# Lumina-Group/libzkp

Measured on AMD Instinct MI355X. Metric: proofs/sec (whole node) + ms/proof p50, 4096-proof mixed batch (range / equality / membership / improvement) per MI355X, higher is better.
Workload: dtype u32/u64 integer limbs (10x25.5-bit GF(2^255-19), BN254 Fq on 9x29-bit limbs in the MSM loops and 10x26-bit elsewhere, 8x32-bit Fr and scalars mod l, 2x64-bit f128)

## Files before the change

__graft_entry__.py:

```python
import ctypes
import os
import re
import subprocess
import sys

ROOT = os.path.dirname(os.path.abspath(__file__))
CSRC = os.path.join(ROOT, "libzkp_amd", "csrc")
LIB = os.path.join(ROOT, "libzkp_amd", "lib", "libzkp_hip.so")
ORACLE_LIB = os.path.join(ROOT, "oracle", "_build", "libzkp_oracle.so")
EMUL_DIR = os.path.join(ROOT, "tests", "emul")


def _newer(target, sources):
    if not os.path.exists(target):
        return False
    t = os.path.getmtime(target)
    return all(os.path.getmtime(s) <= t for s in sources)


def _run(cmd, **kw):
    print("+", " ".join(cmd), flush=True)
    subprocess.check_call(cmd, **kw)


# ... 32 lines not shown
        _run([hipcc, "--offload-arch=gfx950", "-shared", "-pthread", "-o", LIB] + objs)


def build_oracle(force=False):
    cdir = os.path.join(ROOT, "oracle", "c")
    srcs = [os.path.join(cdir, f) for f in os.listdir(cdir)] + [os.path.join(ROOT, "oracle", "Makefile")]
    if not force and _newer(ORACLE_LIB, srcs):
        return
    _run(["make", "-C", os.path.join(ROOT, "oracle"), "clean", "all"])


def build_emul(force=False):
    out = os.path.join(EMUL_DIR, "_build")
    os.makedirs(out, exist_ok=True)
    hdrs = [os.path.join(CSRC, f) for f in os.listdir(CSRC) if f.endswith(".h")]
    for name in ("emul_math", "emul_bp", "emul_bn254", "emul_g16", "emul_stark", "emul_g16_localise"):
        so, src = os.path.join(out, "lib%s.so" % name), os.path.join(EMUL_DIR, name + ".cpp")
        if not force and _newer(so, hdrs + [src]):
            continue
        _run(["g++", "-O2", "-std=c++17", "-fPIC", "-shared", "-o", so, src])


def build_abi_caller(force=False):
    src = os.path.join(ROOT, "tests", "abi", "abi_call_all.cpp")
    out = os.path.join(ROOT, "tests", "abi", "_build")
    exe = os.path.join(out, "abi_call_all")
    os.makedirs(out, exist_ok=True)
    if force or not _newer(exe, [src, os.path.join(ROOT, "include", "libzkp_hip.h"), LIB]):
        _run(["g++", "-O1", "-std=c++17", "-pthread", "-D__HIP_PLATFORM_AMD__", "-I/opt/rocm/include", src, "-o", exe, "-L" + os.path.dirname(LIB), "-lzkp_hip",
              "-L/opt/rocm/lib", "-lamdhip64", "-Wl,-rpath,$ORIGIN/../../../libzkp_amd/lib", "-Wl,-rpath,/opt/rocm/lib"])
    return exe
# ... 78 lines not shown
```

libzkp_amd/csrc/bp_steps.h:

```cpp
#pragma once
#include "fe25519.h"
#include "sc25519.h"
#include "ge25519.h"
#include "keccak.h"

namespace zkp {

constexpr uint32_t BP_N = 64;
constexpr uint32_t BASE_B = 0, BASE_BB = 1, BASE_G = 2, BASE_H = 66, NBASE = 130;
constexpr uint32_t WBITS = 10, NWIN = 26, NENT = 512, DIGW = 13, NWIN_U64 = 7, NIELS_W = 30, SUBTAB_W = NENT * NIELS_W;
constexpr uint32_t TAPE_SLOTS = 132;
constexpr uint32_t P1_V = 0, P1_A = 2, P1_NSLOTS = 260;
constexpr uint32_t P2_NSLOTS = 4;
constexpr uint32_t PR_NSLOTS = 130;
ZKP_HD constexpr uint32_t p1_s(uint32_t n) { return 3 + 2 * n; }
ZKP_HD constexpr uint32_t tape_slots(uint32_t n) { return 2 * n + 4; }
ZKP_HD constexpr uint32_t rp_bytes(uint32_t lg) { return 32 * (9 + 2 * lg); }
constexpr uint32_t GE_W = 40;
enum { SC_Y = 0, SC_Z, SC_X, SC_W, SC_U, SC_UINV, SC_T0, SC_T1, SC_T2, SC_NUM };
enum { KIND_RANGE_MIN = 0, KIND_RANGE_MAX, KIND_THRESHOLD, KIND_CONSISTENCY, KIND_BULLETPROOF, KIND_NUM };

struct BpView {
    uint32_t M;
    uint32_t n, lg;
// ... 11 lines not shown
    uint32_t* tape;
    uint32_t* gamma;
    uint32_t* d1;
    uint32_t* d2;
    uint32_t* dr;
    uint32_t* yinvpow;
    uint32_t* ypq;
    uint32_t* r0;
    uint32_t* r1;
    uint32_t* pp;
    uint32_t* ab;
    uint32_t* gh;
    uint32_t* scal;
    uint32_t* tstate;
    uint32_t* enc;
};

ZKP_HD inline sc ld_sc(const uint32_t* p, uint32_t idx, uint32_t row, uint32_t rows) {
    sc r; const uint32_t* q = p + (size_t)idx * 8 * rows + row;
    ZKP_UNROLL for (int k = 0; k < 8; k++) r.v[k] = q[(size_t)k * rows];
    return r;
}
ZKP_HD inline void st_sc(uint32_t* p, uint32_t idx, uint32_t row, uint32_t rows, const sc& s) {
    uint32_t* q = p + (size_t)idx * 8 * rows + row;
    ZKP_UNROLL for (int k = 0; k < 8; k++) q[(size_t)k * rows] = s.v[k];
}
ZKP_HD inline void st_digits_raw(uint32_t* d, uint32_t slot, uint32_t row, uint32_t rows, const sc& raw, uint32_t wbits = 0) {
    uint32_t* q = d + (size_t)slot * DIGW * rows + row;
    if (wbits == 16) {
        uint32_t pk[8]; sc_recode_signed65536(pk, raw);
// ... 123 lines not shown

ZKP_HD inline void strobe_save(const BpView& V, uint32_t job, const Strobe& s) {
    for (int i = 0; i < 50; i++) V.tstate[(size_t)i * V.M + job] = s.base[i * s.stride];
    V.tstate[(size_t)50 * V.M + job] = s.pos; V.tstate[(size_t)51 * V.M + job] = s.pos_begin;
}
ZKP_HD inline void strobe_load(const BpView& V, uint32_t job, Strobe& s) {
    for (int i = 0; i < 50; i++) s.base[i * s.stride] = V.tstate[(size_t)i * V.M + job];
    s.pos = V.tstate[(size_t)50 * V.M + job]; s.pos_begin = V.tstate[(size_t)51 * V.M + job];
}
ZKP_HD inline sc merlin_challenge_scalar(Strobe& s, const char* label, uint32_t label_len) {
    uint32_t w[16]; merlin_challenge_words(s, label, label_len, w, 16);
    return sc_from_wide(w);
}
ZKP_HD inline void merlin_append_scalar(Strobe& s, const char* label, uint32_t label_len, const sc& raw) { merlin_append_words(s, label, label_len, raw.v, 8); }

ZKP_HD inline void step_transcript1(const BpView& V, uint32_t job, Strobe& s) {
    const uint32_t M = V.M;
    switch (V.kind[job]) {
        case KIND_RANGE_MIN: merlin_init(s, "libzkp_range_min", 16); break;
        case KIND_RANGE_MAX: merlin_init(s, "libzkp_range_max", 16); break;
        case KIND_THRESHOLD: merlin_init(s, "libzkp_threshold", 16); break;
        case KIND_CONSISTENCY: merlin_init(s, "libzkp_consistency", 18); break;
        default: merlin_init(s, "libzkp_bulletproof", 18); break;
    }
    merlin_append_bytes(s, "dom-sep", 7, "rangeproof v1", 13);
    merlin_append_u64(s, "n", 1, V.n);
    merlin_append_u64(s, "m", 1, 1);
    const sc Ve = ld_sc(V.enc, 0, job, M), Ae = ld_sc(V.enc, 1, job, M), Se = ld_sc(V.enc, 2, job, M);
    merlin_append_words(s, "V", 1, Ve.v, 8);
    merlin_append_words(s, "A", 1, Ae.v, 8);
    merlin_append_words(s, "S", 1, Se.v, 8);
    const sc y = merlin_challenge_scalar(s, "y", 1);
    const sc z = merlin_challenge_scalar(s, "z", 1);
    strobe_save(V, job, s);
    st_sc(V.scal, SC_Y, job, M, y);
    st_sc(V.scal, SC_Z, job, M, z);
    const sc yinv = sc_invert(y);
    for (uint32_t h = 0; h < 2; h++) {
        const sc base = h ? yinv : y;
        sc p = sc_one();
        for (uint32_t b = 0; b < 8; b++) { st_sc(V.ypq, 16 * h + b, job, M, p); p = sc_mul(p, base); }
        sc q = sc_one();
        for (uint32_t a = 0; a < 8; a++) { st_sc(V.ypq, 16 * h + 8 + a, job, M, q); q = sc_mul(q, p); }
    }
    uint8_t* pr = V.out + V.proof_off[job];
    put_bytes(pr, Ae.v, 8); put_bytes(pr + 32, Se.v, 8);
    put_bytes(V.out + V.commit_off[job], Ve.v, 8);
}

ZKP_HD inline void step_poly(const BpView& V, uint32_t i, uint32_t job) {
    const uint32_t M = V.M;
    const sc yi = sc_mul(ld_sc(V.ypq, 8 + (i >> 3), job, M), ld_sc(V.ypq, i & 7u, job, M));
    st_sc(V.yinvpow, i, job, M, sc_mul(ld_sc(V.ypq, 24 + (i >> 3), job, M), ld_sc(V.ypq, 16 + (i & 7u), job, M)));
    const sc z = ld_sc(V.scal, SC_Z, job, M);
    const sc zz = sc_mul(z, z);
    const uint32_t bit = (uint32_t)(V.v[job] >> i) & 1u;
    const sc one = sc_one();
    const sc l0 = bit ? sc_sub(one, z) : sc_neg(z);
    const sc arz = bit ? z : sc_sub(z, one);
    const sc two_i = sc_from_u64(1ull << i);
    const sc r0 = sc_add(sc_mul(yi, arz), sc_mul(zz, two_i));
    const sc l1 = ld_sc(V.tape, 2 + i, job, M);
// ... 15 lines not shown
    }
    return t;
}
ZKP_HD inline void step_poly_sum_finish(const BpView& V, uint32_t job, const ScTriple& t) {
    const uint32_t M = V.M;
    const sc t0 = t.a, t2 = t.c, t1 = sc_sub(sc_sub(t.b, t0), t2);
    st_sc(V.scal, SC_T0, job, M, t0); st_sc(V.scal, SC_T1, job, M, t1); st_sc(V.scal, SC_T2, job, M, t2);
    st_digits(V.d2, 0, job, M, t1, V.wbits);
    st_digits(V.d2, 2, job, M, t2, V.wbits);
}
ZKP_HD inline void step_poly_sum(const BpView& V, uint32_t job) {
    ScTriple t = step_poly_sum_part(V, 0, job);
    for (uint32_t p = 1; p < 8; p++) t = triple_add(t, step_poly_sum_part(V, p, job));
    step_poly_sum_finish(V, job, t);
}
ZKP_HD inline void step_transcript2(const BpView& V, uint32_t job, Strobe& s) {
    const uint32_t M = V.M;
    strobe_load(V, job, s);
    const sc T1e = ld_sc(V.enc, 0, job, M), T2e = ld_sc(V.enc, 1, job, M);
    merlin_append_words(s, "T_1", 3, T1e.v, 8);
    merlin_append_words(s, "T_2", 3, T2e.v, 8);
    const sc x = merlin_challenge_scalar(s, "x", 1);
    const sc xx = sc_mul(x, x);
    const sc z = ld_sc(V.scal, SC_Z, job, M), zz = sc_mul(z, z);
    const sc t0 = ld_sc(V.scal, SC_T0, job, M), t1 = ld_sc(V.scal, SC_T1, job, M), t2 = ld_sc(V.scal, SC_T2, job, M);
    const sc t_x = sc_add(sc_add(t0, sc_mul(t1, x)), sc_mul(t2, xx));
    const sc t1_bl = ld_sc(V.tape, 2 + 2 * V.n, job, M), t2_bl = ld_sc(V.tape, 3 + 2 * V.n, job, M);
    const sc t_x_bl = sc_add(sc_add(sc_mul(zz, ld_sc(V.gamma, 0, job, M)), sc_mul(t1_bl, x)), sc_mul(t2_bl, xx));
    const sc e_bl = sc_add(ld_sc(V.tape, 0, job, M), sc_mul(ld_sc(V.tape, 1, job, M), x));
    const sc r_tx = sc_to_raw(t_x), r_txb = sc_to_raw(t_x_bl), r_eb = sc_to_raw(e_bl);
    merlin_append_scalar(s, "t_x", 3, r_tx);
    merlin_append_scalar(s, "t_x_blinding", 12, r_txb);
    merlin_append_scalar(s, "e_blinding", 10, r_eb);
    const sc w = merlin_challenge_scalar(s, "w", 1);
    merlin_append_bytes(s, "dom-sep", 7, "ipp v1", 6);
    merlin_append_u64(s, "n", 1, V.n);
    strobe_save(V, job, s);
    st_sc(V.scal, SC_X, job, M, x); st_sc(V.scal, SC_W, job, M, w);
    uint8_t* pr = V.out + V.proof_off[job];
    put_bytes(pr + 64, T1e.v, 8); put_bytes(pr + 96, T2e.v, 8);
    put_bytes(pr + 128, r_tx.v, 8); put_bytes(pr + 160, r_txb.v, 8); put_bytes(pr + 192, r_eb.v, 8);
}
ZKP_HD inline void step_lr_init(const BpView& V, uint32_t i, uint32_t job) {
    const uint32_t M = V.M;
    const sc z = ld_sc(V.scal, SC_Z, job, M), x = ld_sc(V.scal, SC_X, job, M);
    const uint32_t bit = (uint32_t)(V.v[job] >> i) & 1u;
    const sc l0 = bit ? sc_sub(sc_one(), z) : sc_neg(z);
    const sc a = sc_add(l0, sc_mul(ld_sc(V.tape, 2 + i, job, M), x));
    const sc b = sc_add(ld_sc(V.r0, i, job, M), sc_mul(ld_sc(V.r1, i, job, M), x));
    st_sc(V.ab, i, job, M, a); st_sc(V.ab, 64 + i, job, M, b);
}

ZKP_HD inline void step_round_prep(const BpView& V, uint32_t r, uint32_t i, uint32_t job) {
    const uint32_t M = V.M, p = V.lg - 1 - r, k = 1u << p, half = V.n >> 1;
    const uint32_t* abp = V.ab + (size_t)(r & 1) * (2 * 64 * 8) * M;
    uint32_t* abn = V.ab + (size_t)((r + 1) & 1) * (2 * 64 * 8) * M;
    sc u = sc_one(), uinv = sc_one();
// ... 22 lines not shown
    st_digits(V.dr, bit ? V.n + 2 + half + rank : 1 + half + rank, job, M, sc_mul(bx, h), V.wbits);
    if (i < k) {
        const sc ai = cur_a(i), bi = cur_b(i);
        st_sc(V.pp, i, job, M, sc_mul(ai, bx));
        st_sc(V.pp, 32 + i, job, M, sc_mul(ax, bi));
    }
}
ZKP_HD inline void step_round_sum(const BpView& V, uint32_t r, uint32_t job) {
    const uint32_t M = V.M, k = (V.n >> 1) >> r;
    sc cL = sc_zero(), cR = sc_zero();
    for (uint32_t j = 0; j < k; j++) { cL = sc_add(cL, ld_sc(V.pp, j, job, M)); cR = sc_add(cR, ld_sc(V.pp, 32 + j, job, M)); }
    const sc w = ld_sc(V.scal, SC_W, job, M);
    st_digits(V.dr, 0, job, M, sc_mul(cL, w), V.wbits);
    st_digits(V.dr, V.n + 1, job, M, sc_mul(cR, w), V.wbits);
}
ZKP_HD inline void step_transcript_round(const BpView& V, uint32_t r, uint32_t job, Strobe& s) {
    const uint32_t M = V.M;
    strobe_load(V, job, s);
    const sc Le = ld_sc(V.enc, 0, job, M), Re = ld_sc(V.enc, 1, job, M);
    merlin_append_words(s, "L", 1, Le.v, 8);
    merlin_append_words(s, "R", 1, Re.v, 8);
    const sc u = merlin_challenge_scalar(s, "u", 1);
    const sc uinv = sc_invert(u);
    uint8_t* pr = V.out + V.proof_off[job];
    put_bytes(pr + 224 + 64 * r, Le.v, 8); put_bytes(pr + 256 + 64 * r, Re.v, 8);
    if (r + 1 < V.lg) {
        strobe_save(V, job, s);
        st_sc(V.scal, SC_U, job, M, u); st_sc(V.scal, SC_UINV, job, M, uinv);
    } else {
        const uint32_t* abp = V.ab + (size_t)(V.lg & 1u) * (2 * 64 * 8) * M;
        const sc a = sc_add(sc_mul(ld_sc(abp, 0, job, M), u), sc_mul(ld_sc(abp, 1, job, M), uinv));
        const sc b = sc_add(sc_mul(ld_sc(abp, 64, job, M), uinv), sc_mul(ld_sc(abp, 65, job, M), u));
        const sc ra = sc_to_raw(a), rb = sc_to_raw(b);
        put_bytes(pr + 224 + 64 * V.lg, ra.v, 8); put_bytes(pr + 256 + 64 * V.lg, rb.v, 8);
    }
}

struct CtView {
    uint32_t C;
    const uint64_t* v; const uint32_t* seed_ix; const uint32_t* bl_ix; const uint32_t* seeds;
    uint32_t* digits;
    uint32_t wbits = 0;
};
ZKP_HD inline void step_ctask(const CtView& T, uint32_t c) {
    uint32_t seed[8]; const uint32_t* p = T.seeds + (size_t)T.seed_ix[c] * 8;
    ZKP_UNROLL for (int k = 0; k < 8; k++) seed[k] = p[k];
    const uint64_t v = T.v[c];
    st_digits_raw(T.digits, 0, c, T.C, sc_words((uint32_t)v, (uint32_t)(v >> 32), 0, 0, 0, 0, 0, 0), T.wbits);
    st_digits(T.digits, 1, c, T.C, tape_blinding(seed, T.bl_ix[c]), T.wbits);
}
// ... 40 lines not shown
```

libzkp_amd/csrc/zkp_hip.hip:

```cpp
#include <hip/hip_runtime.h>
#include <mutex>
#include <memory>
#include <algorithm>
#include <map>
#include <array>
#include <type_traits>
#include <atomic>
#include <thread>
#include <condition_variable>
#include <functional>
#include <deque>
#include <new>
#include <exception>
#include <cstring>
#include <string>
#include <vector>
#include <cstdio>
#include <cstdlib>
#include <cmath>
#include <chrono>
#include <sys/random.h>
#include "bp_layout.h"
#include "g16_steps.h"
#include "sha256_host.h"
// ... 59 lines not shown
__global__ void __launch_bounds__(TB) k_lr_init(BpView V) {
    ZKP_RAISE_PRIO();
    const uint32_t job = blockIdx.x * TB + threadIdx.x;
    if (job < V.M) step_lr_init(V, blockIdx.y, job);
}
__global__ void __launch_bounds__(TB, LAT_WAVES) k_round_prep(BpView V, uint32_t r) {
    ZKP_RAISE_PRIO();
    const uint32_t job = blockIdx.x * TB + threadIdx.x;
    if (job < V.M) step_round_prep(V, r, blockIdx.y, job);
}
__global__ void __launch_bounds__(TW, LAT_WAVES) k_round_sum(BpView V, uint32_t r) {
    ZKP_RAISE_PRIO();
    const uint32_t job = blockIdx.x * TW + threadIdx.x;
    if (job < V.M) step_round_sum(V, r, job);
}
__global__ void __launch_bounds__(TW, 1) k_transcript1(BpView V) {
    ZKP_RAISE_PRIO();
    __shared__ uint32_t lds[50 * TW];
    const uint32_t job = blockIdx.x * TW + threadIdx.x;
    Strobe s; s.base = lds + threadIdx.x; s.stride = TW; s.pos = 0; s.pos_begin = 0;
    if (job < V.M) step_transcript1(V, job, s);
}
__global__ void __launch_bounds__(TW, 1) k_transcript2(BpView V) {
    ZKP_RAISE_PRIO();
    __shared__ uint32_t lds[50 * TW];
    const uint32_t job = blockIdx.x * TW + threadIdx.x;
    Strobe s; s.base = lds + threadIdx.x; s.stride = TW; s.pos = 0; s.pos_begin = 0;
    if (job < V.M) step_transcript2(V, job, s);
}
__global__ void __launch_bounds__(TW, 1) k_transcript_round(BpView V, uint32_t r) {
    ZKP_RAISE_PRIO();
    __shared__ uint32_t lds[50 * TW];
    const uint32_t job = blockIdx.x * TW + threadIdx.x;
    Strobe s; s.base = lds + threadIdx.x; s.stride = TW; s.pos = 0; s.pos_begin = 0;
    if (job < V.M) step_transcript_round(V, r, job, s);
}
__global__ void __launch_bounds__(TW, 1) k_encode(ReduceView R, const uint32_t* sums) {
    ZKP_RAISE_PRIO();
    const uint32_t row = blockIdx.x * TW + threadIdx.x, target = blockIdx.y;
    if (row >= R.rows) return;
    sc e; ge_ristretto_encode(e.v, ld_ge(sums, target, row, R.rows));
    st_sc(R.enc, target, row, R.rows, e);
    if (R.out_off != nullptr && target == 0) put_bytes(R.out + R.out_off[row], e.v, 8);
}

struct EdMsm {
    static constexpr uint32_t ACC_W = GE_W;
    using Acc = ge;
    static __device__ __forceinline__ Acc identity() { return ge_identity(); }
    static __device__ __forceinline__ void store(uint32_t* p, uint32_t idx, uint32_t row, uint32_t rows, const Acc& a) { st_ge(p, idx, row, rows, a); }
// ... 118 lines not shown
};
constexpr uint32_t NSLOTS = 2;

struct G16State; struct StarkState; struct VfyState; struct BatchState;
struct Device {
    int index = 0, hip_dev = 0;
    std::mutex mu;
    bool ready = false;
    uint64_t generation = 0;
    int num_cu = 256;
    int msm_prio_now = 0;
    hipStream_t stream = nullptr;
    uint32_t* d_edg_table = nullptr;
    EdgGeom edg = {0, 0, 0, 0, 0};
    bool bp_ready = false;
    int edg_blocks_per_cu = 3;
    struct Family { LayoutSet p1, rd[6]; bool ready = false; };
    Family fam[4];
    LayoutSet p2, ct;
    uint32_t max_chunks = 0;
    SubBatch sub[NSLOTS];
    uint32_t next_slot = 0;
    DevPool pool;
    G16State* g16 = nullptr; StarkState* stark = nullptr; VfyState* vfy = nullptr; BatchState* batch = nullptr;
    bool profiling = false;
    struct KProf {
        std::vector<std::pair<hipEvent_t, hipEvent_t>> ev_pool; size_t ev_used = 0;
        double ms = 0; uint64_t launches = 0, adds = 0;
    };
    KProf prof[3];
// ... 290 lines not shown
    drop();
    D.edg = g;
    R.v.push_back({D.hip_dev, D.d_edg_table, 1, g});
    return 0;
}
int ensure_bp() {
    Device& D = dev();
    if (D.bp_ready) return 0;
    int rc;
    if ((rc = build_edg_table())) return rc;
    D.max_chunks = 0;
    if ((rc = upload_set(D.p2, targets_phase2((uint8_t)D.edg.nwin)))) return rc;
    if ((rc = upload_set(D.ct, targets_ctask((uint8_t)D.edg.nwin, (uint8_t)D.edg.nwin_u64)))) return rc;
    D.max_chunks = D.p2.max_chunks;
    if ((rc = ensure_family(6))) return rc;
    D.bp_ready = true;
    return 0;
}

int init_device() {
    Device& D = dev();
    if (D.ready) return 0;
    bool lazy = false;
    int rc = ed_tables_lazy(&lazy);
    if (rc) return rc;
    hipDeviceProp_t prop; HIP_TRY(hipGetDeviceProperties(&prop, D.hip_dev));
    D.num_cu = prop.multiProcessorCount > 0 ? prop.multiProcessorCount : 256;
    if (!D.stream) HIP_TRY(hipStreamCreateWithFlags(&D.stream, hipStreamNonBlocking));
    if (!lazy && (rc = ensure_bp())) return rc;
    D.ready = true;
// ... 102 lines not shown
    uint64_t* ct_off;
    int* flag;
};
size_t align_up(size_t x) { return (x + 255) & ~(size_t)255; }

size_t carve(uint8_t* base, uint32_t M, uint32_t C, uint32_t max_chunks, Ws* w) {
    size_t off = 0;
    auto take = [&](size_t bytes) { uint8_t* p = base ? base + off : nullptr; off += align_up(bytes); return p; };
    const size_t W = (size_t)8 * 4 * M;
    const size_t WD = (size_t)DIGW * 4 * M;
    Ws t{};
    t.J.v = (uint64_t*)take(8ull * M); t.J.seed_ix = (uint32_t*)take(4ull * M); t.J.proof_ix = (uint32_t*)take(4ull * M);
    t.J.bl_plus = (int32_t*)take(4ull * M); t.J.bl_minus = (int32_t*)take(4ull * M); t.J.kind = (uint8_t*)take(M);
    t.J.proof_off = (uint64_t*)take(8ull * M); t.J.commit_off = (uint64_t*)take(8ull * M);
    t.J.ct_v = (uint64_t*)take(8ull * C); t.J.ct_seed_ix = (uint32_t*)take(4ull * C); t.J.ct_bl_ix = (uint32_t*)take(4ull * C); t.J.ct_off = (uint64_t*)take(8ull * C);
    t.V.wbits = dev().edg.wbits; t.T.wbits = dev().edg.wbits;
    t.V.M = M; t.V.v = t.J.v; t.V.seed_ix = t.J.seed_ix; t.V.proof_ix = t.J.proof_ix; t.V.bl_plus = t.J.bl_plus; t.V.bl_minus = t.J.bl_minus;
    t.V.kind = t.J.kind; t.V.proof_off = t.J.proof_off; t.V.commit_off = t.J.commit_off;
    t.V.tape = (uint32_t*)take(W * TAPE_SLOTS); t.V.gamma = (uint32_t*)take(W);
    t.V.d1 = (uint32_t*)take(WD * P1_NSLOTS); t.V.d2 = (uint32_t*)take(WD * P2_NSLOTS); t.V.dr = (uint32_t*)take(WD * PR_NSLOTS);
    t.V.yinvpow = (uint32_t*)take(W * 64); t.V.ypq = (uint32_t*)take(W * 32); t.V.r0 = (uint32_t*)take(W * 64); t.V.r1 = (uint32_t*)take(W * 64);
    t.V.pp = (uint32_t*)take(W * 192); t.V.ab = (uint32_t*)take(W * 256); t.V.gh = (uint32_t*)take(W * 128);
    t.V.scal = (uint32_t*)take(W * SC_NUM); t.V.tstate = (uint32_t*)take(4ull * 52 * M); t.V.enc = (uint32_t*)take(W * 3);
    t.partial = (uint32_t*)take((size_t)max_chunks * GE_W * 4 * M);
    t.sums = (uint32_t*)take((size_t)3 * GE_W * 4 * M);
    t.T.C = C; t.T.v = t.J.ct_v; t.T.seed_ix = t.J.ct_seed_ix; t.T.bl_ix = t.J.ct_bl_ix;
    t.T.digits = (uint32_t*)take((size_t)2 * DIGW * 4 * C);
    t.ct_partial = (uint32_t*)take((size_t)(dev().ct.max_chunks ? dev().ct.max_chunks : 2) * GE_W * 4 * C);
    t.ct_enc = (uint32_t*)take((size_t)8 * 4 * C);
    t.ct_sums = (uint32_t*)take((size_t)GE_W * 4 * C);
    t.ct_off = t.J.ct_off;
// ... 35 lines not shown
    ReduceView R; R.rows = rows; R.ntargets = D.ntargets; R.partial = partial; R.target_chunk_begin = D.target_chunk_begin;
    R.enc = enc; R.out_off = out_off; R.out = out; R.corr = nullptr;
    ZKP_TRACED("k_sum_t<EdMsm>", st, launch_sum_ed(R, sums, st));
    ZKP_TRACED("k_encode", st, k_encode<<<dim3((rows + TW - 1) / TW, D.ntargets), TW, 0, st>>>(R, sums));
    return 0;
}
int msm_and_encode(const LayoutSet& S, uint32_t rows, const uint32_t* digits, uint32_t* partial, uint32_t* sums, uint32_t* enc, const uint64_t* out_off, uint8_t* out, hipStream_t st) {
    const DevLayout& D = pick_layout(S, rows);
    int rc = launch_msm(D, rows, digits, partial, st);
    if (rc) return rc;
    return launch_reduce(D, rows, partial, sums, enc, out_off, out, st);
}

int run_pipeline(const Ws& w, uint32_t M, uint32_t C, hipStream_t st, SubBatch& lane) {
    int rc;
    const dim3 gj((M + TB - 1) / TB), gw((M + TW - 1) / TW);
    const uint32_t n = w.V.n, lg = w.V.lg;
    const Device::Family& F = dev().fam[lg - 3];
    const bool forked = C != 0 && M != 0;
    if (C) {
        hipStream_t cs = forked ? lane.side : st;
        if (forked) { HIP_TRY(hipEventRecord(lane.side_go, st)); HIP_TRY(hipStreamWaitEvent(cs, lane.side_go, 0)); }
        ZKP_TRACED("k_ctask", cs, k_ctask<<<(C + TB - 1) / TB, TB, 0, cs>>>(w.T));
        if ((rc = msm_and_encode(dev().ct, C, w.T.digits, w.ct_partial, w.ct_sums, w.ct_enc, w.ct_off, w.V.out, cs))) return rc;
        if (forked) HIP_TRY(hipEventRecord(lane.side_done, cs));
    }
    if (M == 0) { HIP_TRY(hipGetLastError()); return 0; }
    ZKP_TRACED("k_tape", st, k_tape<<<dim3(gj.x, tape_slots(n) + 1), TB, 0, st>>>(w.V));
    if ((rc = msm_and_encode(F.p1, M, w.V.d1, w.partial, w.sums, w.V.enc, nullptr, nullptr, st))) return rc;
    ZKP_TRACED("k_transcript1", st, k_transcript1<<<gw, TW, 0, st>>>(w.V));
    ZKP_TRACED("k_poly", st, k_poly<<<dim3(gj.x, n), TB, 0, st>>>(w.V));
    ZKP_TRACED("k_poly_sum", st, k_poly_sum<<<(M + 7) / 8, TW, 0, st>>>(w.V));
    if ((rc = msm_and_encode(dev().p2, M, w.V.d2, w.partial, w.sums, w.V.enc, nullptr, nullptr, st))) return rc;
    ZKP_TRACED("k_transcript2", st, k_transcript2<<<gw, TW, 0, st>>>(w.V));
    ZKP_TRACED("k_lr_init", st, k_lr_init<<<dim3(gj.x, n), TB, 0, st>>>(w.V));
    for (uint32_t r = 0; r < lg; r++) {
        ZKP_TRACED("k_round_prep", st, k_round_prep<<<dim3(gj.x, n), TB, 0, st>>>(w.V, r));
        ZKP_TRACED("k_round_sum", st, k_round_sum<<<gw, TW, 0, st>>>(w.V, r));
        if ((rc = msm_and_encode(F.rd[r], M, w.V.dr, w.partial, w.sums, w.V.enc, nullptr, nullptr, st))) return rc;
        ZKP_TRACED("k_transcript_round", st, k_transcript_round<<<gw, TW, 0, st>>>(w.V, r));
    }
    if (forked) HIP_TRY(hipStreamWaitEvent(st, lane.side_done, 0));
    HIP_TRY(hipGetLastError());
    return 0;
}

__global__ void k_any_failed(const int32_t* status, uint32_t n, int* flag) {
    const uint32_t i = blockIdx.x * blockDim.x + threadIdx.x;
    if (i < n && status[i] != 0) atomicOr(flag, 1);
}

int prove_range_device_locked(uint64_t n, const uint64_t* d_value, const uint64_t* d_min, const uint64_t* d_max, uint32_t lg,
                              const uint8_t* d_seeds, uint8_t* d_out, uint64_t stride, uint32_t* d_out_len, int32_t* d_status,
                              hipStream_t st, int* any_failed, int slot_hint = -1) {
    if (n == 0) { if (any_failed) *any_failed = 0; return 0; }
// ... 234 lines not shown
    t_sel = 0;
    for (Device* d : shards) {
        std::lock_guard<std::mutex> lk(d->mu);
        if (!d->ready) continue;
        Device* prev = t_dev; t_dev = d;
        (void)hipSetDevice(d->hip_dev);
        (void)hipDeviceSynchronize();
        batch_release_all();
        g16_release_all();
        bpv_release_all();
        stark_release_all();
        d->pool.release_all();
        for (auto& sb : d->sub) release_sub(sb);
        d->msm_prio_now = 0;
        release_edg_table();
        free_set(d->p2); free_set(d->ct);
        for (auto& F : d->fam) { free_set(F.p1); for (auto& s : F.rd) free_set(s); F.ready = false; }
        trace_release();
        for (auto& K : d->prof) { for (auto& e : K.ev_pool) { (void)hipEventDestroy(e.first); (void)hipEventDestroy(e.second); } K = Device::KProf(); }
        d->g16_verify = Device::G16VerifyStats();
        (void)hipStreamDestroy(d->stream); d->stream = nullptr;
        d->ready = false; d->bp_ready = false; d->profiling = false; d->max_chunks = 0; d->next_slot = 0; d->generation++;
        t_dev = prev;
    }
} ZKP_API_CATCH_VOID

void zkp_hip_profile_enable(int on) try {
    std::vector<Device*> shards;
    { Registry& R = registry(); std::lock_guard<std::mutex> lk(R.mu); shards = R.shards; }
    for (Device* d : shards) { std::lock_guard<std::mutex> dl(d->mu); d->profiling = on != 0; }
// ... 131 lines not shown
```

Before: 329,500.

## Run Bulletproof Merlin transcripts cooperatively across 32 lanes per job

Replaces the one-thread-per-job Strobe/Keccak transcript kernels with a cooperative version. Each job's 25-lane Keccak state is spread across 32 lanes of a wave using ds_bpermute shuffles, and the scalar tails (inversions, powers, proof writes) are then done by one thread per job from shared memory. It also precomputes the fixed transcript prefix per kind and size on the host and loads it instead of re-absorbing it. This targets the serial, LDS-heavy per-thread Keccak latency in the transcript steps. In exchange it uses many more threads per job and adds block syncs and some idle lanes during the tails.

```diff
diff --git a/__graft_entry__.py b/__graft_entry__.py
--- a/__graft_entry__.py
+++ b/__graft_entry__.py
@@ -70,7 +70,7 @@
     out = os.path.join(EMUL_DIR, "_build")
     os.makedirs(out, exist_ok=True)
     hdrs = [os.path.join(CSRC, f) for f in os.listdir(CSRC) if f.endswith(".h")]
-    for name in ("emul_math", "emul_bp", "emul_bn254", "emul_g16", "emul_stark", "emul_g16_localise"):
+    for name in ("emul_math", "emul_bp", "emul_bn254", "emul_g16", "emul_stark", "emul_g16_localise", "emul_transcript_lanes"):
         so, src = os.path.join(out, "lib%s.so" % name), os.path.join(EMUL_DIR, name + ".cpp")
         if not force and _newer(so, hdrs + [src]):
             continue
diff --git a/libzkp_amd/csrc/bp_steps.h b/libzkp_amd/csrc/bp_steps.h
--- a/libzkp_amd/csrc/bp_steps.h
+++ b/libzkp_amd/csrc/bp_steps.h
@@ -3,6 +3,7 @@
 #include "sc25519.h"
 #include "ge25519.h"
 #include "keccak.h"
+#include "keccak_lanes.h"
 
 namespace zkp {
 
@@ -49,6 +50,7 @@
     uint32_t* scal;
     uint32_t* tstate;
     uint32_t* enc;
+    const uint32_t* tprefix = nullptr;
 };
 
 ZKP_HD inline sc ld_sc(const uint32_t* p, uint32_t idx, uint32_t row, uint32_t rows) {
@@ -202,9 +204,8 @@
 }
 ZKP_HD inline void merlin_append_scalar(Strobe& s, const char* label, uint32_t label_len, const sc& raw) { merlin_append_words(s, label, label_len, raw.v, 8); }
 
-ZKP_HD inline void step_transcript1(const BpView& V, uint32_t job, Strobe& s) {
-    const uint32_t M = V.M;
-    switch (V.kind[job]) {
+ZKP_HD inline void transcript_prefix(Strobe& s, uint32_t kind, uint32_t n) {
+    switch (kind) {
         case KIND_RANGE_MIN: merlin_init(s, "libzkp_range_min", 16); break;
         case KIND_RANGE_MAX: merlin_init(s, "libzkp_range_max", 16); break;
         case KIND_THRESHOLD: merlin_init(s, "libzkp_threshold", 16); break;
@@ -212,15 +213,22 @@
         default: merlin_init(s, "libzkp_bulletproof", 18); break;
     }
     merlin_append_bytes(s, "dom-sep", 7, "rangeproof v1", 13);
-    merlin_append_u64(s, "n", 1, V.n);
+    merlin_append_u64(s, "n", 1, n);
     merlin_append_u64(s, "m", 1, 1);
-    const sc Ve = ld_sc(V.enc, 0, job, M), Ae = ld_sc(V.enc, 1, job, M), Se = ld_sc(V.enc, 2, job, M);
-    merlin_append_words(s, "V", 1, Ve.v, 8);
-    merlin_append_words(s, "A", 1, Ae.v, 8);
-    merlin_append_words(s, "S", 1, Se.v, 8);
-    const sc y = merlin_challenge_scalar(s, "y", 1);
-    const sc z = merlin_challenge_scalar(s, "z", 1);
-    strobe_save(V, job, s);
+}
+constexpr uint32_t TPREFIX_W = 52, TPREFIX_N = KIND_NUM * 4;
+ZKP_HD inline uint32_t tprefix_entry(uint32_t kind, uint32_t lg) { return (kind < KIND_NUM ? kind : (uint32_t)KIND_BULLETPROOF) * 4 + (lg - 3); }
+inline void host_build_tprefix(uint32_t out[TPREFIX_N * TPREFIX_W]) {
+    for (uint32_t kind = 0; kind < KIND_NUM; kind++) for (uint32_t lg = 3; lg <= 6; lg++) {
+        uint32_t* e = out + (size_t)tprefix_entry(kind, lg) * TPREFIX_W;
+        Strobe s; s.base = e; s.stride = 1; s.pos = 0; s.pos_begin = 0;
+        transcript_prefix(s, kind, 1u << lg);
+        e[50] = s.pos; e[51] = s.pos_begin;
+    }
+}
+ZKP_HD inline void transcript1_tail(const BpView& V, uint32_t job, const uint32_t* ch) {
+    const uint32_t M = V.M;
+    const sc y = sc_from_wide(ch), z = sc_from_wide(ch + 16);
     st_sc(V.scal, SC_Y, job, M, y);
     st_sc(V.scal, SC_Z, job, M, z);
     const sc yinv = sc_invert(y);
@@ -231,9 +239,33 @@
         sc q = sc_one();
         for (uint32_t a = 0; a < 8; a++) { st_sc(V.ypq, 16 * h + 8 + a, job, M, q); q = sc_mul(q, p); }
     }
+    const sc Ve = ld_sc(V.enc, 0, job, M), Ae = ld_sc(V.enc, 1, job, M), Se = ld_sc(V.enc, 2, job, M);
     uint8_t* pr = V.out + V.proof_off[job];
     put_bytes(pr, Ae.v, 8); put_bytes(pr + 32, Se.v, 8);
     put_bytes(V.out + V.commit_off[job], Ve.v, 8);
+}
+ZKP_HD inline void step_transcript1(const BpView& V, uint32_t job, Strobe& s) {
+    const uint32_t M = V.M;
+    transcript_prefix(s, V.kind[job], V.n);
+    const sc Ve = ld_sc(V.enc, 0, job, M), Ae = ld_sc(V.enc, 1, job, M), Se = ld_sc(V.enc, 2, job, M);
+    merlin_append_words(s, "V", 1, Ve.v, 8);
+    merlin_append_words(s, "A", 1, Ae.v, 8);
+    merlin_append_words(s, "S", 1, Se.v, 8);
+    uint32_t ch[32];
+    merlin_challenge_words(s, "y", 1, ch, 16);
+    merlin_challenge_words(s, "z", 1, ch + 16, 16);
+    strobe_save(V, job, s);
+    transcript1_tail(V, job, ch);
+}
+template <class P> ZKP_HD inline void coop_transcript1_sponge(const BpView& V, uint32_t job, uint32_t* ch) {
+    const size_t M = V.M;
+    KlStrobe<P> s; kl_load(s, V.tprefix + (size_t)tprefix_entry(V.kind[job], V.lg) * TPREFIX_W, 1);
+    kl_append(s, "V", 1, KlWords{V.enc + job, M}, 32);
+    kl_append(s, "A", 1, KlWords{V.enc + 8 * M + job, M}, 32);
+    kl_append(s, "S", 1, KlWords{V.enc + 16 * M + job, M}, 32);
+    kl_challenge(s, "y", 1, (uint8_t*)ch, 64);
+    kl_challenge(s, "z", 1, (uint8_t*)(ch + 16), 64);
+    kl_save(s, V.tstate + job, M);
 }
 
 ZKP_HD inline void step_poly(const BpView& V, uint32_t i, uint32_t job) {
@@ -279,13 +311,10 @@
     for (uint32_t p = 1; p < 8; p++) t = triple_add(t, step_poly_sum_part(V, p, job));
     step_poly_sum_finish(V, job, t);
 }
-ZKP_HD inline void step_transcript2(const BpView& V, uint32_t job, Strobe& s) {
-    const uint32_t M = V.M;
-    strobe_load(V, job, s);
+ZKP_HD inline void transcript2_tail(const BpView& V, uint32_t job, const uint32_t* ch, uint32_t* raw) {
+    const uint32_t M = V.M;
     const sc T1e = ld_sc(V.enc, 0, job, M), T2e = ld_sc(V.enc, 1, job, M);
-    merlin_append_words(s, "T_1", 3, T1e.v, 8);
-    merlin_append_words(s, "T_2", 3, T2e.v, 8);
-    const sc x = merlin_challenge_scalar(s, "x", 1);
+    const sc x = sc_from_wide(ch);
     const sc xx = sc_mul(x, x);
     const sc z = ld_sc(V.scal, SC_Z, job, M), zz = sc_mul(z, z);
     const sc t0 = ld_sc(V.scal, SC_T0, job, M), t1 = ld_sc(V.scal, SC_T1, job, M), t2 = ld_sc(V.scal, SC_T2, job, M);
@@ -294,18 +323,47 @@
     const sc t_x_bl = sc_add(sc_add(sc_mul(zz, ld_sc(V.gamma, 0, job, M)), sc_mul(t1_bl, x)), sc_mul(t2_bl, xx));
     const sc e_bl = sc_add(ld_sc(V.tape, 0, job, M), sc_mul(ld_sc(V.tape, 1, job, M), x));
     const sc r_tx = sc_to_raw(t_x), r_txb = sc_to_raw(t_x_bl), r_eb = sc_to_raw(e_bl);
-    merlin_append_scalar(s, "t_x", 3, r_tx);
-    merlin_append_scalar(s, "t_x_blinding", 12, r_txb);
-    merlin_append_scalar(s, "e_blinding", 10, r_eb);
+    ZKP_UNROLL for (int k = 0; k < 8; k++) { raw[k] = r_tx.v[k]; raw[8 + k] = r_txb.v[k]; raw[16 + k] = r_eb.v[k]; }
+    st_sc(V.scal, SC_X, job, M, x);
+    uint8_t* pr = V.out + V.proof_off[job];
+    put_bytes(pr + 64, T1e.v, 8); put_bytes(pr + 96, T2e.v, 8);
+    put_bytes(pr + 128, r_tx.v, 8); put_bytes(pr + 160, r_txb.v, 8); put_bytes(pr + 192, r_eb.v, 8);
+}
+ZKP_HD inline void step_transcript2(const BpView& V, uint32_t job, Strobe& s) {
+    const uint32_t M = V.M;
+    strobe_load(V, job, s);
+    const sc T1e = ld_sc(V.enc, 0, job, M), T2e = ld_sc(V.enc, 1, job, M);
+    merlin_append_words(s, "T_1", 3, T1e.v, 8);
+    merlin_append_words(s, "T_2", 3, T2e.v, 8);
+    uint32_t ch[16], raw[24];
+    merlin_challenge_words(s, "x", 1, ch, 16);
+    transcript2_tail(V, job, ch, raw);
+    merlin_append_words(s, "t_x", 3, raw, 8);
+    merlin_append_words(s, "t_x_blinding", 12, raw + 8, 8);
+    merlin_append_words(s, "e_blinding", 10, raw + 16, 8);
     const sc w = merlin_challenge_scalar(s, "w", 1);
     merlin_append_bytes(s, "dom-sep", 7, "ipp v1", 6);
     merlin_append_u64(s, "n", 1, V.n);
     strobe_save(V, job, s);
-    st_sc(V.scal, SC_X, job, M, x); st_sc(V.scal, SC_W, job, M, w);
-    uint8_t* pr = V.out + V.proof_off[job];
-    put_bytes(pr + 64, T1e.v, 8); put_bytes(pr + 96, T2e.v, 8);
-    put_bytes(pr + 128, r_tx.v, 8); put_bytes(pr + 160, r_txb.v, 8); put_bytes(pr + 192, r_eb.v, 8);
-}
+    st_sc(V.scal, SC_W, job, M, w);
+}
+template <class P> ZKP_HD inline void coop_transcript2_sponge_a(const BpView& V, uint32_t job, KlStrobe<P>& s, uint32_t* ch) {
+    const size_t M = V.M;
+    kl_load(s, V.tstate + job, M);
+    kl_append(s, "T_1", 3, KlWords{V.enc + job, M}, 32);
+    kl_append(s, "T_2", 3, KlWords{V.enc + 8 * M + job, M}, 32);
+    kl_challenge(s, "x", 1, (uint8_t*)ch, 64);
+}
+template <class P> ZKP_HD inline void coop_transcript2_sponge_b(const BpView& V, uint32_t job, KlStrobe<P>& s, const uint32_t* raw, uint32_t* ch) {
+    kl_append(s, "t_x", 3, KlWords{raw, 1}, 32);
+    kl_append(s, "t_x_blinding", 12, KlWords{raw + 8, 1}, 32);
+    kl_append(s, "e_blinding", 10, KlWords{raw + 16, 1}, 32);
+    kl_challenge(s, "w", 1, (uint8_t*)ch, 64);
+    kl_append_str(s, "dom-sep", 7, "ipp v1", 6);
+    kl_append_u64(s, "n", 1, V.n);
+    kl_save(s, V.tstate + job, (size_t)V.M);
+}
+ZKP_HD inline void transcript2_finish(const BpView& V, uint32_t job, const uint32_t* ch) { st_sc(V.scal, SC_W, job, V.M, sc_from_wide(ch)); }
 ZKP_HD inline void step_lr_init(const BpView& V, uint32_t i, uint32_t job) {
     const uint32_t M = V.M;
     const sc z = ld_sc(V.scal, SC_Z, job, M), x = ld_sc(V.scal, SC_X, job, M);
@@ -358,18 +416,14 @@
     st_digits(V.dr, 0, job, M, sc_mul(cL, w), V.wbits);
     st_digits(V.dr, V.n + 1, job, M, sc_mul(cR, w), V.wbits);
 }
-ZKP_HD inline void step_transcript_round(const BpView& V, uint32_t r, uint32_t job, Strobe& s) {
-    const uint32_t M = V.M;
-    strobe_load(V, job, s);
+ZKP_HD inline void transcript_round_tail(const BpView& V, uint32_t r, uint32_t job, const uint32_t* ch) {
+    const uint32_t M = V.M;
     const sc Le = ld_sc(V.enc, 0, job, M), Re = ld_sc(V.enc, 1, job, M);
-    merlin_append_words(s, "L", 1, Le.v, 8);
-    merlin_append_words(s, "R", 1, Re.v, 8);
-    const sc u = merlin_challenge_scalar(s, "u", 1);
+    const sc u = sc_from_wide(ch);
     const sc uinv = sc_invert(u);
     uint8_t* pr = V.out + V.proof_off[job];
     put_bytes(pr + 224 + 64 * r, Le.v, 8); put_bytes(pr + 256 + 64 * r, Re.v, 8);
     if (r + 1 < V.lg) {
-        strobe_save(V, job, s);
         st_sc(V.scal, SC_U, job, M, u); st_sc(V.scal, SC_UINV, job, M, uinv);
     } else {
         const uint32_t* abp = V.ab + (size_t)(V.lg & 1u) * (2 * 64 * 8) * M;
@@ -378,6 +432,25 @@
         const sc ra = sc_to_raw(a), rb = sc_to_raw(b);
         put_bytes(pr + 224 + 64 * V.lg, ra.v, 8); put_bytes(pr + 256 + 64 * V.lg, rb.v, 8);
     }
+}
+ZKP_HD inline void step_transcript_round(const BpView& V, uint32_t r, uint32_t job, Strobe& s) {
+    const uint32_t M = V.M;
+    strobe_load(V, job, s);
+    const sc Le = ld_sc(V.enc, 0, job, M), Re = ld_sc(V.enc, 1, job, M);
+    merlin_append_words(s, "L", 1, Le.v, 8);
+    merlin_append_words(s, "R", 1, Re.v, 8);
+    uint32_t ch[16];
+    merlin_challenge_words(s, "u", 1, ch, 16);
+    if (r + 1 < V.lg) strobe_save(V, job, s);
+    transcript_round_tail(V, r, job, ch);
+}
+template <class P> ZKP_HD inline void coop_transcript_round_sponge(const BpView& V, uint32_t r, uint32_t job, uint32_t* ch) {
+    const size_t M = V.M;
+    KlStrobe<P> s; kl_load(s, V.tstate + job, M);
+    kl_append(s, "L", 1, KlWords{V.enc + job, M}, 32);
+    kl_append(s, "R", 1, KlWords{V.enc + 8 * M + job, M}, 32);
+    kl_challenge(s, "u", 1, (uint8_t*)ch, 64);
+    if (r + 1 < V.lg) kl_save(s, V.tstate + job, M);
 }
 
 struct CtView {
diff --git a/libzkp_amd/csrc/keccak_lanes.h b/libzkp_amd/csrc/keccak_lanes.h
--- /dev/null
+++ b/libzkp_amd/csrc/keccak_lanes.h
@@ -0,0 +1,158 @@
+#pragma once
+#include "keccak.h"
+
+namespace zkp {
+
+ZKP_HD inline uint64_t kl_rol(uint64_t x, uint32_t n) { return (x << n) | (x >> ((64 - n) & 63)); }
+
+template <class P> ZKP_HD inline typename P::U64 kl_keccak_f1600(typename P::U64 a) {
+    using U64 = typename P::U64;
+    const uint64_t RC[24] = {
+        0x0000000000000001ULL, 0x0000000000008082ULL, 0x800000000000808AULL, 0x8000000080008000ULL,
+        0x000000000000808BULL, 0x0000000080000001ULL, 0x8000000080008081ULL, 0x8000000000008009ULL,
+        0x000000000000008AULL, 0x0000000000000088ULL, 0x0000000080008009ULL, 0x000000008000000AULL,
+        0x000000008000808BULL, 0x800000000000008BULL, 0x8000000000008089ULL, 0x8000000000008003ULL,
+        0x8000000000008002ULL, 0x8000000000000080ULL, 0x000000000000800AULL, 0x800000008000000AULL,
+        0x8000000080008081ULL, 0x8000000000008080ULL, 0x0000000080000001ULL, 0x8000000080008008ULL};
+    for (int r = 0; r < 24; r++) {
+        const U64 s1 = P::shfl(a, [](uint32_t i) { return (i + 5) % 25; }), s2 = P::shfl(a, [](uint32_t i) { return (i + 10) % 25; });
+        const U64 s3 = P::shfl(a, [](uint32_t i) { return (i + 15) % 25; }), s4 = P::shfl(a, [](uint32_t i) { return (i + 20) % 25; });
+        const U64 c = P::map([](uint32_t, uint64_t v, uint64_t p, uint64_t q, uint64_t s, uint64_t t) { return v ^ p ^ q ^ s ^ t; }, a, s1, s2, s3, s4);
+        const U64 cm = P::shfl(c, [](uint32_t i) { return (i + 4) % 5; }), cp = P::shfl(c, [](uint32_t i) { return (i + 1) % 5; });
+        a = P::map([](uint32_t, uint64_t v, uint64_t m, uint64_t p) { return v ^ m ^ kl_rol(p, 1); }, a, cm, cp);
+        U64 b = P::shfl(a, [](uint32_t i) {
+            const uint8_t src[32] = {0, 6, 12, 18, 24, 3, 9, 10, 16, 22, 1, 7, 13, 19, 20, 4, 5, 11, 17, 23, 2, 8, 14, 15, 21, 0, 0, 0, 0, 0, 0, 0};
+            return (uint32_t)src[i];
+        });
+        b = P::map([](uint32_t i, uint64_t v) {
+            const uint8_t rot[32] = {0, 44, 43, 21, 14, 28, 20, 3, 45, 61, 1, 6, 25, 8, 18, 27, 36, 10, 15, 56, 62, 55, 39, 41, 2, 0, 0, 0, 0, 0, 0, 0};
+            return kl_rol(v, rot[i]);
+        }, b);
+        const U64 b1 = P::shfl(b, [](uint32_t i) { return i < 25 ? i - i % 5 + (i % 5 + 1) % 5 : 0u; });
+        const U64 b2 = P::shfl(b, [](uint32_t i) { return i < 25 ? i - i % 5 + (i % 5 + 2) % 5 : 0u; });
+        const uint64_t rc = RC[r];
+        a = P::map([rc](uint32_t i, uint64_t v, uint64_t p, uint64_t q) { return v ^ (~p & q) ^ (i == 0 ? rc : 0); }, b, b1, b2);
+    }
+    return a;
+}
+
+template <class P> struct KlStrobe { typename P::U64 a; uint32_t pos, pos_begin; };
+
+ZKP_HD inline uint64_t kl_xor_byte(uint64_t a, uint32_t lane, uint32_t pos, uint32_t byte) { return (pos >> 3) == lane ? a ^ ((uint64_t)byte << (8 * (pos & 7))) : a; }
+ZKP_HD inline uint64_t kl_byte_mask(uint32_t b0, uint32_t b1) { return (b1 == 8 ? ~0ull : (1ull << (8 * b1)) - 1) & ~((1ull << (8 * b0)) - 1); }
+
+template <class P> ZKP_HD inline void kl_run_f(KlStrobe<P>& s) {
+    const uint32_t pos = s.pos, pb = s.pos_begin;
+    s.a = P::map([pos, pb](uint32_t lane, uint64_t a) {
+        a = kl_xor_byte(a, lane, pos, pb); a = kl_xor_byte(a, lane, pos + 1, 0x04);
+        return kl_xor_byte(a, lane, STROBE_R + 1, 0x80);
+    }, s.a);
+    s.a = kl_keccak_f1600<P>(s.a);
+    s.pos = 0; s.pos_begin = 0;
+}
+template <class P, class W> ZKP_HD inline void kl_absorb(KlStrobe<P>& s, W word, uint32_t len) {
+    const int32_t nw = (int32_t)((len + 3) >> 2);
+    for (uint32_t done = 0; done < len;) {
+        const uint32_t pos = s.pos, left = len - done, room = STROBE_R - pos, take = left < room ? left : room;
+        s.a = P::map([&word, pos, take, done, nw](uint32_t lane, uint64_t a) {
+            const uint32_t w0 = 8 * lane, lo = w0 > pos ? w0 : pos, hi = w0 + 8 < pos + take ? w0 + 8 : pos + take;
+            if (lo >= hi) return a;
+            const int32_t j0 = (int32_t)(w0 + done) - (int32_t)pos;
+            const int32_t k0 = j0 >> 2; const uint32_t sh = 8 * ((uint32_t)j0 & 3u);
+            auto w = [&word, nw](int32_t k) -> uint64_t { return k >= 0 && k < nw ? (uint64_t)word((uint32_t)k) : 0; };
+            const uint64_t low = w(k0) | (w(k0 + 1) << 32);
+            const uint64_t win = sh ? (low >> sh) | (w(k0 + 2) << (64 - sh)) : low;
+            return a ^ (win & kl_byte_mask(lo - w0, hi - w0));
+        }, s.a);
+        s.pos += take; done += take;
+        if (s.pos == STROBE_R) kl_run_f(s);
+    }
+}
+template <class P> ZKP_HD inline void kl_squeeze(KlStrobe<P>& s, uint8_t* out, uint32_t len) {
+    for (uint32_t done = 0; done < len;) {
+        const uint32_t pos = s.pos, left = len - done, room = STROBE_R - pos, take = left < room ? left : room;
+        s.a = P::map([out, pos, take, done](uint32_t lane, uint64_t a) {
+            const uint32_t w0 = 8 * lane, lo = w0 > pos ? w0 : pos, hi = w0 + 8 < pos + take ? w0 + 8 : pos + take;
+            if (lo >= hi) return a;
+            for (uint32_t p = lo; p < hi; p++) out[done + (p - pos)] = (uint8_t)(a >> (8 * (p - w0)));
+            return a & ~kl_byte_mask(lo - w0, hi - w0);
+        }, s.a);
+        s.pos += take; done += take;
+        if (s.pos == STROBE_R) kl_run_f(s);
+    }
+}
+template <class P> ZKP_HD inline void kl_begin_op(KlStrobe<P>& s, uint32_t flags) {
+    const uint32_t two = s.pos_begin | (flags << 8);
+    s.pos_begin = s.pos + 1;
+    kl_absorb(s, [two](uint32_t) { return two; }, 2);
+    if ((flags & (STROBE_FLAG_C | STROBE_FLAG_K)) && s.pos != 0) kl_run_f(s);
+}
+
+struct KlPack4 {
+    uint32_t w[4];
+    ZKP_HD uint32_t operator()(uint32_t k) const { return k == 0 ? w[0] : k == 1 ? w[1] : k == 2 ? w[2] : w[3]; }
+};
+ZKP_HD inline KlPack4 kl_pack(const char* str, uint32_t len, bool with_suffix, uint32_t suffix) {
+    KlPack4 p; p.w[0] = p.w[1] = p.w[2] = p.w[3] = 0;
+    ZKP_UNROLL for (uint32_t i = 0; i < 16; i++) {
+        uint32_t byte = 0;
+        if (i < len) byte = (uint8_t)str[i];
+        else if (with_suffix && i < len + 4) byte = (suffix >> (8 * (i - len))) & 0xffu;
+        p.w[i >> 2] |= byte << (8 * (i & 3));
+    }
+    return p;
+}
+struct KlWords { const uint32_t* p; size_t stride; ZKP_HD uint32_t operator()(uint32_t k) const { return p[(size_t)k * stride]; } };
+
+template <class P> ZKP_HD inline void kl_begin_append(KlStrobe<P>& s, const char* label, uint32_t label_len, uint32_t msg_len) {
+    kl_begin_op(s, STROBE_FLAG_M | STROBE_FLAG_A);
+    kl_absorb(s, kl_pack(label, label_len, true, msg_len), label_len + 4);
+    kl_begin_op(s, STROBE_FLAG_A);
+}
+template <class P, class W> ZKP_HD inline void kl_append(KlStrobe<P>& s, const char* label, uint32_t label_len, W word, uint32_t msg_len) {
+    kl_begin_append(s, label, label_len, msg_len);
+    kl_absorb(s, word, msg_len);
+}
+template <class P> ZKP_HD inline void kl_append_str(KlStrobe<P>& s, const char* label, uint32_t label_len, const char* msg, uint32_t msg_len) {
+    kl_append(s, label, label_len, kl_pack(msg, msg_len, false, 0), msg_len);
+}
+template <class P> ZKP_HD inline void kl_append_u64(KlStrobe<P>& s, const char* label, uint32_t label_len, uint64_t x) {
+    KlPack4 p; p.w[0] = (uint32_t)x; p.w[1] = (uint32_t)(x >> 32); p.w[2] = p.w[3] = 0;
+    kl_append(s, label, label_len, p, 8);
+}
+template <class P> ZKP_HD inline void kl_challenge(KlStrobe<P>& s, const char* label, uint32_t label_len, uint8_t* out, uint32_t len) {
+    kl_begin_op(s, STROBE_FLAG_M | STROBE_FLAG_A);
+    kl_absorb(s, kl_pack(label, label_len, true, len), label_len + 4);
+    kl_begin_op(s, STROBE_FLAG_I | STROBE_FLAG_A | STROBE_FLAG_C);
+    kl_squeeze(s, out, len);
+}
+template <class P> ZKP_HD inline void kl_load(KlStrobe<P>& s, const uint32_t* p, size_t stride) {
+    s.a = P::map([p, stride](uint32_t lane) -> uint64_t {
+        if (lane >= 25) return 0;
+        return (uint64_t)p[(size_t)(2 * lane) * stride] | ((uint64_t)p[(size_t)(2 * lane + 1) * stride] << 32);
+    });
+    s.pos = p[50 * stride]; s.pos_begin = p[51 * stride];
+}
+template <class P> ZKP_HD inline void kl_save(const KlStrobe<P>& s, uint32_t* p, size_t stride) {
+    const uint32_t pos = s.pos, pb = s.pos_begin;
+    P::map([p, stride, pos, pb](uint32_t lane, uint64_t a) -> uint64_t {
+        if (lane < 25) { p[(size_t)(2 * lane) * stride] = (uint32_t)a; p[(size_t)(2 * lane + 1) * stride] = (uint32_t)(a >> 32); }
+        if (lane == 25) { p[50 * stride] = pos; p[51 * stride] = pb; }
+        return a;
+    }, s.a);
+}
+
+#if defined(__HIPCC__)
+struct WaveLanes {
+    using U64 = uint64_t;
+    template <class F, class... A> __device__ static __forceinline__ U64 map(F f, A... a) { return f(threadIdx.x & 31u, a...); }
+    template <class S> __device__ static __forceinline__ U64 shfl(U64 v, S src) {
+        const int addr = (int)(((threadIdx.x & 32u) | src(threadIdx.x & 31u)) << 2);
+        const uint32_t lo = (uint32_t)__builtin_amdgcn_ds_bpermute(addr, (int)(uint32_t)v);
+        const uint32_t hi = (uint32_t)__builtin_amdgcn_ds_bpermute(addr, (int)(uint32_t)(v >> 32));
+        return (uint64_t)lo | ((uint64_t)hi << 32);
+    }
+};
+#endif
+
+}
diff --git a/libzkp_amd/csrc/zkp_hip.hip b/libzkp_amd/csrc/zkp_hip.hip
--- a/libzkp_amd/csrc/zkp_hip.hip
+++ b/libzkp_amd/csrc/zkp_hip.hip
@@ -97,26 +97,36 @@
     const uint32_t job = blockIdx.x * TW + threadIdx.x;
     if (job < V.M) step_round_sum(V, r, job);
 }
-__global__ void __launch_bounds__(TW, 1) k_transcript1(BpView V) {
+static constexpr uint32_t TJ = 8, TT = 32 * TJ;
+__global__ void __launch_bounds__(TT, 1) k_transcript1(BpView V) {
     ZKP_RAISE_PRIO();
-    __shared__ uint32_t lds[50 * TW];
-    const uint32_t job = blockIdx.x * TW + threadIdx.x;
-    Strobe s; s.base = lds + threadIdx.x; s.stride = TW; s.pos = 0; s.pos_begin = 0;
-    if (job < V.M) step_transcript1(V, job, s);
-}
-__global__ void __launch_bounds__(TW, 1) k_transcript2(BpView V) {
+    __shared__ uint32_t ch[TJ][32];
+    const uint32_t g = threadIdx.x >> 5, job = blockIdx.x * TJ + g, tail_job = blockIdx.x * TJ + threadIdx.x;
+    if (job < V.M) coop_transcript1_sponge<WaveLanes>(V, job, ch[g]);
+    __syncthreads();
+    if (threadIdx.x < TJ && tail_job < V.M) transcript1_tail(V, tail_job, ch[threadIdx.x]);
+}
+__global__ void __launch_bounds__(TT, 1) k_transcript2(BpView V) {
     ZKP_RAISE_PRIO();
-    __shared__ uint32_t lds[50 * TW];
-    const uint32_t job = blockIdx.x * TW + threadIdx.x;
-    Strobe s; s.base = lds + threadIdx.x; s.stride = TW; s.pos = 0; s.pos_begin = 0;
-    if (job < V.M) step_transcript2(V, job, s);
-}
-__global__ void __launch_bounds__(TW, 1) k_transcript_round(BpView V, uint32_t r) {
+    __shared__ uint32_t ch[TJ][16], raw[TJ][24];
+    const uint32_t g = threadIdx.x >> 5, job = blockIdx.x * TJ + g, tail_job = blockIdx.x * TJ + threadIdx.x;
+    const bool tail = threadIdx.x < TJ && tail_job < V.M;
+    KlStrobe<WaveLanes> s; s.a = 0; s.pos = 0; s.pos_begin = 0;
+    if (job < V.M) coop_transcript2_sponge_a(V, job, s, ch[g]);
+    __syncthreads();
+    if (tail) transcript2_tail(V, tail_job, ch[threadIdx.x], raw[threadIdx.x]);
+    __syncthreads();
+    if (job < V.M) coop_transcript2_sponge_b(V, job, s, raw[g], ch[g]);
+    __syncthreads();
+    if (tail) transcript2_finish(V, tail_job, ch[threadIdx.x]);
+}
+__global__ void __launch_bounds__(TT, 1) k_transcript_round(BpView V, uint32_t r) {
     ZKP_RAISE_PRIO();
-    __shared__ uint32_t lds[50 * TW];
-    const uint32_t job = blockIdx.x * TW + threadIdx.x;
-    Strobe s; s.base = lds + threadIdx.x; s.stride = TW; s.pos = 0; s.pos_begin = 0;
-    if (job < V.M) step_transcript_round(V, r, job, s);
+    __shared__ uint32_t ch[TJ][16];
+    const uint32_t g = threadIdx.x >> 5, job = blockIdx.x * TJ + g, tail_job = blockIdx.x * TJ + threadIdx.x;
+    if (job < V.M) coop_transcript_round_sponge<WaveLanes>(V, r, job, ch[g]);
+    __syncthreads();
+    if (threadIdx.x < TJ && tail_job < V.M) transcript_round_tail(V, r, tail_job, ch[threadIdx.x]);
 }
 __global__ void __launch_bounds__(TW, 1) k_encode(ReduceView R, const uint32_t* sums) {
     ZKP_RAISE_PRIO();
@@ -265,6 +275,7 @@
     uint32_t* d_edg_table = nullptr;
     EdgGeom edg = {0, 0, 0, 0, 0};
     bool bp_ready = false;
+    uint32_t* d_tprefix = nullptr;
     int edg_blocks_per_cu = 3;
     struct Family { LayoutSet p1, rd[6]; bool ready = false; };
     Family fam[4];
@@ -585,6 +596,12 @@
     if ((rc = upload_set(D.ct, targets_ctask((uint8_t)D.edg.nwin, (uint8_t)D.edg.nwin_u64)))) return rc;
     D.max_chunks = D.p2.max_chunks;
     if ((rc = ensure_family(6))) return rc;
+    if (!D.d_tprefix) {
+        std::vector<uint32_t> tp((size_t)TPREFIX_N * TPREFIX_W);
+        host_build_tprefix(tp.data());
+        HIP_TRY(hipMalloc(&D.d_tprefix, tp.size() * 4));
+        HIP_TRY(hipMemcpy(D.d_tprefix, tp.data(), tp.size() * 4, hipMemcpyHostToDevice));
+    }
     D.bp_ready = true;
     return 0;
 }
@@ -717,7 +734,7 @@
     t.J.bl_plus = (int32_t*)take(4ull * M); t.J.bl_minus = (int32_t*)take(4ull * M); t.J.kind = (uint8_t*)take(M);
     t.J.proof_off = (uint64_t*)take(8ull * M); t.J.commit_off = (uint64_t*)take(8ull * M);
     t.J.ct_v = (uint64_t*)take(8ull * C); t.J.ct_seed_ix = (uint32_t*)take(4ull * C); t.J.ct_bl_ix = (uint32_t*)take(4ull * C); t.J.ct_off = (uint64_t*)take(8ull * C);
-    t.V.wbits = dev().edg.wbits; t.T.wbits = dev().edg.wbits;
+    t.V.wbits = dev().edg.wbits; t.T.wbits = dev().edg.wbits; t.V.tprefix = dev().d_tprefix;
     t.V.M = M; t.V.v = t.J.v; t.V.seed_ix = t.J.seed_ix; t.V.proof_ix = t.J.proof_ix; t.V.bl_plus = t.J.bl_plus; t.V.bl_minus = t.J.bl_minus;
     t.V.kind = t.J.kind; t.V.proof_off = t.J.proof_off; t.V.commit_off = t.J.commit_off;
     t.V.tape = (uint32_t*)take(W * TAPE_SLOTS); t.V.gamma = (uint32_t*)take(W);
@@ -783,7 +800,7 @@
 
 int run_pipeline(const Ws& w, uint32_t M, uint32_t C, hipStream_t st, SubBatch& lane) {
     int rc;
-    const dim3 gj((M + TB - 1) / TB), gw((M + TW - 1) / TW);
+    const dim3 gj((M + TB - 1) / TB), gw((M + TW - 1) / TW), gt((M + TJ - 1) / TJ);
     const uint32_t n = w.V.n, lg = w.V.lg;
     const Device::Family& F = dev().fam[lg - 3];
     const bool forked = C != 0 && M != 0;
@@ -797,17 +814,17 @@
     if (M == 0) { HIP_TRY(hipGetLastError()); return 0; }
     ZKP_TRACED("k_tape", st, k_tape<<<dim3(gj.x, tape_slots(n) + 1), TB, 0, st>>>(w.V));
     if ((rc = msm_and_encode(F.p1, M, w.V.d1, w.partial, w.sums, w.V.enc, nullptr, nullptr, st))) return rc;
-    ZKP_TRACED("k_transcript1", st, k_transcript1<<<gw, TW, 0, st>>>(w.V));
+    ZKP_TRACED("k_transcript1", st, k_transcript1<<<gt, TT, 0, st>>>(w.V));
     ZKP_TRACED("k_poly", st, k_poly<<<dim3(gj.x, n), TB, 0, st>>>(w.V));
     ZKP_TRACED("k_poly_sum", st, k_poly_sum<<<(M + 7) / 8, TW, 0, st>>>(w.V));
     if ((rc = msm_and_encode(dev().p2, M, w.V.d2, w.partial, w.sums, w.V.enc, nullptr, nullptr, st))) return rc;
-    ZKP_TRACED("k_transcript2", st, k_transcript2<<<gw, TW, 0, st>>>(w.V));
+    ZKP_TRACED("k_transcript2", st, k_transcript2<<<gt, TT, 0, st>>>(w.V));
     ZKP_TRACED("k_lr_init", st, k_lr_init<<<dim3(gj.x, n), TB, 0, st>>>(w.V));
     for (uint32_t r = 0; r < lg; r++) {
         ZKP_TRACED("k_round_prep", st, k_round_prep<<<dim3(gj.x, n), TB, 0, st>>>(w.V, r));
         ZKP_TRACED("k_round_sum", st, k_round_sum<<<gw, TW, 0, st>>>(w.V, r));
         if ((rc = msm_and_encode(F.rd[r], M, w.V.dr, w.partial, w.sums, w.V.enc, nullptr, nullptr, st))) return rc;
-        ZKP_TRACED("k_transcript_round", st, k_transcript_round<<<gw, TW, 0, st>>>(w.V, r));
+        ZKP_TRACED("k_transcript_round", st, k_transcript_round<<<gt, TT, 0, st>>>(w.V, r));
     }
     if (forked) HIP_TRY(hipStreamWaitEvent(st, lane.side_done, 0));
     HIP_TRY(hipGetLastError());
@@ -1072,6 +1089,7 @@
         for (auto& sb : d->sub) release_sub(sb);
         d->msm_prio_now = 0;
         release_edg_table();
+        (void)hipFree(d->d_tprefix); d->d_tprefix = nullptr;
         free_set(d->p2); free_set(d->ct);
         for (auto& F : d->fam) { free_set(F.p1); for (auto& s : F.rd) free_set(s); F.ready = false; }
         trace_release();
```

Result: no change. 327,000, median of 2 (-0.8%).
